# scychon/openmm_drudeNose

Hardware: AMD Instinct MI355X
Metric: integrator steps/sec at 1M Drude pairs (higher is better)
Workload: dtype f64; 1 GPU; SWM4-NDP water box, 1000000 molecules = 5000000 particle slots, 1000000 Drude pairs, 1 temperature group (+ molecular-COM and Drude thermostats), TGNH mode, mixed precision, numNHChains=1, hard wall 0.02 nm, harness force call-out inside the timed region (harness_force: lattice); harness_force=lattice, precision=mixed, variant=resident, hipgraph=False, parallelism=particle-sharded x1 (whole molecules), one KE all-reduce per step, slots_per_gpu=5000000

## Files before the change

### openmm_drudenose_amd/csrc/tgnh_context.h

```cpp
#ifndef TGNH_CONTEXT_H_
#define TGNH_CONTEXT_H_

#include <map>
#include <string>
#include <vector>

#include "tgnh_internal.h"
#include "tgnh_by_index.h"
#include "tgnh_minimize.h"

void tgnh_set_error(const std::string& msg);

namespace tgnh {
template <typename T> class DeviceBuf {
    T* p_ = nullptr;
    bool pinned_ = false;
public:
    DeviceBuf() = default;
    DeviceBuf(DeviceBuf&& o) noexcept : p_(o.p_), pinned_(o.pinned_) { o.p_ = nullptr; }
    DeviceBuf& operator=(DeviceBuf&& o) noexcept {
        if (this != &o) { reset(); p_ = o.p_; pinned_ = o.pinned_; o.p_ = nullptr; }
        return *this;
    }
    ~DeviceBuf() { reset(); }
// ... 24 lines not shown
    tgnh_status ensure(int grid, bool zero, const char* too_small);
};
}

struct tgnh_context {
    tgnh_desc d;
    int device = 0;
    bool host_only = false;
    struct Topology {
        std::vector<double> mass;
        std::vector<int> pair_drude, pair_parent, group, resid, normal;
        std::vector<int> res_count, res_first;
        std::vector<int> tile_start, tile_res;
        std::vector<int2> res_entries;
        std::vector<int> big_first, big_count;
        int num_big = 0, num_tiles = 0;
        std::vector<uint32_t> meta;
        std::vector<int2> wave_tile;
        std::vector<uint32_t> wmeta;
        std::vector<uint32_t> tile_pat, wtile_pat;
        std::vector<uint32_t> pattern, wpattern;
        std::vector<double> wpat_mass;
        bool wpat_all_uniform = false;
        int num_wtiles = 0;
        tgnh::DeviceBuf<uint32_t> d_meta, d_wmeta, d_tile_pat, d_pattern, d_wpattern;
        tgnh::DeviceBuf<int> d_tile_start, d_tile_res;
        tgnh::DeviceBuf<int2> d_res_table, d_wave_tile, d_big_table;
        tgnh::DeviceBytes d_big_com;
    } topo;
    struct Gather {
        bool generic = false;
        bool chain = false;
        std::string reason;
        std::vector<int2> res_table;
        std::vector<int> resid, partner;
        int com_lanes = 64;
        tgnh::DeviceBuf<int> d_group, d_resid, d_partner;
        tgnh::DeviceBuf<int2> d_res_table;
        tgnh::DeviceBytes d_com;
        tgnh::DeviceBuf<double> d_scratch;
    } gather;
    struct ByIndex {
        tgnh::DeviceBuf<int> d_partner;
    } by_index;
    tgnh::RowScratch<tgnh::DrudeStatsRow> dstats;
    struct CmMotion : tgnh::RowScratch<tgnh::CmRow> {
// ... 140 lines not shown
        tgnh::DeviceBuf<double> d_partials;
        tgnh::DeviceBuf<double> d_state;
        tgnh::DeviceBuf<double> d_stage;
        tgnh::DeviceBuf<double> d_scalar;
    } thermo;
    struct LaunchConfig {
        int grid = 0, gb = 1;
        int num_cus = 256, grid_override = 0;
        std::map<int, int> grid_cache;
        bool alternate_sweeps = true;
        int inline_sum_rows = tgnh::CHAIN_INLINE_SUM_ROWS;
        bool inline_sum_all = false;
        bool carry_ok = false;
        bool inline_chain = false;
        bool wave_ke = false;
        int resident_grid[5][2] = {{0, 0}, {0, 0}, {0, 0}, {0, 0}, {0, 0}};
        int resident_share = 1;
        int wresident_per_cu = 0, wresident_grid = 0;
        int resident_per_cu = 0;
    } cfg;
    struct VelPlanes {
        tgnh::DeviceBytes d_planes;
        tgnh::DeviceBytes d_invm;
        tgnh::DeviceBuf<uint32_t> d_mismatch;
        int verdict = 0;
        int streak = 0;
        bool pinned = false;
        hipStream_t stream = nullptr;
        bool usable() const { return d_planes.get() != nullptr && verdict >= 0 && !pinned; }
    } vp;
    struct Owed {
        bool end_pending = false;
        bool scale_pending = false;
        bool kick_pending = false;
        bool first_half_done = false;
        bool chain_pending = false;
        bool sum_pending = false;
        bool xwait_pending = false;
        bool stage_pending = false;
        bool ke_carry = false;
        bool planes_live = false;
        bool chain_pending_twice = false;
        bool carry_pending = false;
        bool tail_summed = false;
        bool end_folded = false;
        bool g_com_fresh = false;
// ... 80 lines not shown
```

### openmm_drudenose_amd/csrc/tgnh_internal.h

```cpp
#ifndef TGNH_INTERNAL_H_
#define TGNH_INTERNAL_H_

#include <hip/hip_runtime.h>
#include <stdint.h>
#include <type_traits>

#include "../../include/drude_tgnh.h"

namespace tgnh {

#ifndef TGNH_SPT
#define TGNH_SPT 2
#endif
#ifndef TGNH_TBLOCK
#define TGNH_TBLOCK 256
#endif
constexpr int BLOCK = 256;
constexpr int TBLOCK = TGNH_TBLOCK;
constexpr int SPT = TGNH_SPT;
constexpr int TILE_SLOTS = TBLOCK * SPT;
constexpr int TILE_RES = TILE_SLOTS / 2;
constexpr int GRID_CAP = 2048;
constexpr int MAX_GROUPS = 32;

// ... 116 lines not shown
    int num_wtiles;
    int tail_sum;
    double* ke_red;
    int num_tiles;
    int reverse;
    int padded;
    int num_groups;
    int use_com;
    int hardwall;
    double dt;
    double max_dist;
    double hw_scale;
    int chain_on;
    int sum_rows;
    int commit_len, commit_skip, commit_skip_n;
    const double* commit_src;
    double* commit_dst;
    int x_wait;
    const double* st_in;
    double* st_out;
    ChainArgs chain;
    void* vplanes;
    const void* wpat_invm;
};

struct BigComArgs {
    const int2* table;
    int n;
    const void* velm;
    const long long* force;
    int padded;
    int kick;
    double dt;
    void* big_com;
    double* partials;
    int NT, G;
};

struct ForceArgs {
    const void* posq;
    const void* posq_corr;
    const void* x0;
    const uint32_t* meta;
    long long* force;
    int n, padded;
    int reverse;
// ... 78 lines not shown
```

### openmm_drudenose_amd/csrc/tgnh_lifecycle.cpp

```cpp
#include <memory>

#include "tgnh_host.h"
#ifndef TGNH_MEETING_MEM
#define TGNH_MEETING_MEM hipDeviceMallocFinegrained
#endif

static thread_local std::string g_err;
extern "C" const char* tgnh_last_error(void) { return g_err.c_str(); }
extern "C" int tgnh_abi_version(void) { return TGNH_ABI_VERSION; }

void tgnh_set_error(const std::string& msg) { g_err = msg; }

static tgnh_status validate_desc(const tgnh_desc* d, bool* long_chain) {
    if (d->struct_size != sizeof(tgnh_desc)) return fail(TGNH_ERR_ARG, "tgnh_desc size mismatch (ABI)");
    if (d->mode != TGNH_MODE_DUALNH && d->mode != TGNH_MODE_TGNH) return fail(TGNH_ERR_ARG, "bad mode");
    if (d->precision < TGNH_PREC_SINGLE || d->precision > TGNH_PREC_DOUBLE) return fail(TGNH_ERR_ARG, "bad precision");
    if (d->num_particles < 1 || d->num_pairs < 0 || !d->mass || (d->num_pairs && (!d->pair_drude || !d->pair_parent)))
        return fail(TGNH_ERR_ARG, "bad particle / pair arrays");
    if (d->padded_num_particles < d->num_particles) return fail(TGNH_ERR_ARG, "padded_num_particles < num_particles");
    if (d->num_constraints < 0) return fail(TGNH_ERR_ARG, "negative num_constraints");
    if (3LL * d->padded_num_particles > 2147483647LL)
        return fail(TGNH_ERR_UNSUPPORTED, "more than 715 827 882 padded particle slots: the index into the third force plane leaves 32 bits");
    if (d->num_nh_chains < 1 || d->drude_steps_per_real_step < 1) return fail(TGNH_ERR_ARG, "numNHChains and drudeStepsPerRealStep must be >= 1");
    if (d->mode == TGNH_MODE_TGNH && (d->num_groups < 1 || d->num_residues < 1 || !d->group || !d->resid))
// ... 107 lines not shown
}

static tgnh_status resident_census(tgnh_context* c) {
    if (!(c->d.flags & TGNH_FLAG_RESIDENT_STEP) || c->cfg.gb == 0 || !c->cfg.inline_chain || c->thermo.L.NT > CHAIN_INLINE_SUM_NT) return TGNH_OK;
    const int kind = pass_kind(c->d);
    const size_t lds = tile_lds_bytes(c->d.precision, step_kind_ops2(kind), true, true);
    tgnh_status rc = census(c, c->thermo.L.C == 1 ? step_blocks_per_cu(c->d.precision, c->cfg.gb, kind, lds) : 0,
                            [&](const TileArgs& a, int grid) { return launch_step(c->d.precision, c->cfg.gb, kind, a, grid, lds, (hipStream_t)0); },
                            &c->cfg.resident_per_cu);
    if (rc) return rc;
    const bool multi = c->thermo.L.C > 1;
    bool want_w = c->cfg.wave_ke && (c->d.flags & TGNH_FLAG_DEFER_SCALE) && (c->cfg.resident_per_cu > 0 || multi);
    if (c->d.mode == TGNH_MODE_DUALNH && !c->thermo.L.use_drude_chains && multi) want_w = false;
#ifdef TGNH_TUNING
    if (const char* e = getenv("TGNH_WSTEP")) want_w = want_w && e[0] != '0';
#endif
    return census(c, want_w ? wstep_blocks_per_cu(c->d.precision, c->cfg.gb, multi) : 0,
                  [&](const TileArgs& a, int grid) { return launch_wstep(c->d.precision, c->cfg.gb, multi, a, grid, (hipStream_t)0); },
                  &c->cfg.wresident_per_cu);
}

static tgnh_status allocate_velocity_planes(tgnh_context* c) {
    if (const char* e = getenv("TGNH_VELOCITY_PLANES")) if (e[0] == '0') return TGNH_OK;
    if (!(c->d.flags & TGNH_FLAG_DEFER_SCALE) || c->cfg.wresident_per_cu <= 0 || !c->topo.wpat_all_uniform) return TGNH_OK;
    if (c->d.precision == TGNH_PREC_SINGLE) return TGNH_OK;
    if (wstep_blocks_per_cu(c->d.precision, c->cfg.gb, c->thermo.L.C > 1, true) < c->cfg.wresident_per_cu) return TGNH_OK;
    const bool single = c->d.precision == TGNH_PREC_SINGLE;
    const size_t word = single ? sizeof(float) : sizeof(double), n = c->topo.wpat_mass.size();
    std::vector<double> inv(n);
    for (size_t k = 0; k < n; k++) inv[k] = c->topo.wpat_mass[k] == 0.0 ? 0.0 : 1.0 / c->topo.wpat_mass[k];
    std::vector<float> inv_f(inv.begin(), inv.end());
    HIP_OK(c->vp.d_invm.upload(reinterpret_cast<const unsigned char*>(single ? (const void*)inv_f.data() : (const void*)inv.data()), n * word));
    HIP_OK(c->vp.d_mismatch.alloc(1, true));
    HIP_OK(c->vp.d_planes.alloc(3 * (size_t)c->d.padded_num_particles * word, true));
    return TGNH_OK;
}

extern "C" tgnh_status tgnh_create(const tgnh_desc* d, tgnh_handle* out) {
    if (!d || !out) return fail(TGNH_ERR_ARG, "null argument");
    bool long_chain = false;
    tgnh_status rc = validate_desc(d, &long_chain); if (rc) return rc;
    const bool host_only = d->device == -1;
    if (!host_only) {
        int ndev = 0;
        HIP_OK(hipGetDeviceCount(&ndev));
        if (d->device < 0 || d->device >= ndev) return fail(TGNH_ERR_HIP, "no such HIP device (the HIP path needs an MI355X; there is no CPU fallback)");
        HIP_OK(hipSetDevice(d->device));
    }

    std::unique_ptr<tgnh_context> owner(new tgnh_context());
    tgnh_context* c = owner.get();
    c->host_only = host_only;
    c->d = *d;
    c->device = d->device;
    set_bath_temperatures(c, d->temperature, d->drude_temperature);
    make_layout(c);
    c->cfg.gb = c->thermo.L.G <= 1 ? 1 : (c->thermo.L.G <= 4 ? 4 : (c->thermo.L.G <= 8 ? 8 : 0));
// ... 132 lines not shown
```

### openmm_drudenose_amd/csrc/tgnh_queries.cpp

```cpp
#include "tgnh_host.h"

static tgnh_status read_state(tgnh_handle h, int off, int n, hipStream_t s, double* out) {
    if (!out) return fail(TGNH_ERR_ARG, "null out");
    if (h->host_only) { std::copy(h->thermo.h_state.begin() + off, h->thermo.h_state.begin() + off + n, out); return TGNH_OK; }
    { tgnh_status rc = entry(h, false); if (rc) return rc; }
    { tgnh_status rc = materialize_chain(h, s); if (rc) return rc; }
    HIP_OK(hipMemcpyAsync(out, h->thermo.d_state + off, sizeof(double) * n, hipMemcpyDeviceToHost, s));
    return finish_query(h, s);
}

extern "C" tgnh_status tgnh_get_kinetic_energy(tgnh_handle h, int ke_sum_valid, void* stream, double* out) {
    CHECK_H(h);
    if (!out) return fail(TGNH_ERR_ARG, "null out");
    hipStream_t s = (hipStream_t)stream;
    if (h->d.mode == TGNH_MODE_TGNH && ke_sum_valid)
        return read_state(h, h->thermo.L.off_kesum, 1, s, out);
    tgnh_status rc = entry(h, true); if (rc) return rc;
    rc = flush_impl(h, s); if (rc) return rc;
    const double ts = h->d.mode == TGNH_MODE_DUALNH ? 0.5 * h->d.step_size : 0.0;
    HIP_OK(launch_plain_ke(h->d.precision, h->bound.velm, reinterpret_cast<const long long*>(h->bound.force), h->d.num_particles,
                           h->d.padded_num_particles, ts, h->thermo.d_scalar, s));
    HIP_OK(hipMemcpyAsync(out, h->thermo.d_scalar, sizeof(double), hipMemcpyDeviceToHost, s));
    HIP_OK(hipStreamSynchronize(s));
    return TGNH_OK;
// ... 77 lines not shown
        case 0: return &h->topo.normal;
        case 1: return &h->topo.pair_drude;
        case 2: return &h->topo.pair_parent;
        case 3: return &h->topo.group;
        case 4: return &h->topo.resid;
        case 5: return &h->topo.res_count;
        case 6: return &h->topo.res_first;
        case 7: return &h->topo.tile_start;
        default: return nullptr;
    }
}
extern "C" tgnh_status tgnh_get_topology_len(tgnh_handle h, int which, int* len) {
    CHECK_H(h);
    if (!len) return fail(TGNH_ERR_ARG, "null out");
    if (which == 8) { *len = (int)h->topo.meta.size(); return TGNH_OK; }
    if (which == 9) { *len = 2 * (int)h->topo.wave_tile.size(); return TGNH_OK; }
    if (which == 10) { *len = (int)h->topo.wmeta.size(); return TGNH_OK; }
    if (which == 11) { *len = (int)h->topo.tile_pat.size(); return TGNH_OK; }
    if (which == 12) { *len = (int)h->topo.wtile_pat.size(); return TGNH_OK; }
    if (which == 13) { *len = (int)h->topo.pattern.size(); return TGNH_OK; }
    if (which == 14) { *len = (int)h->topo.wpattern.size(); return TGNH_OK; }
    if (which == 15) { *len = 2 * (int)h->topo.wpat_mass.size(); return TGNH_OK; }
    if (which == 16) { *len = 1; return TGNH_OK; }
    const std::vector<int>* v = topo_vec(h, which);
    if (!v) return fail(TGNH_ERR_ARG, "bad topology array id");
    *len = (int)v->size();
    return TGNH_OK;
}
extern "C" tgnh_status tgnh_get_topology(tgnh_handle h, int which, int32_t* out) {
    CHECK_H(h);
    if (!out) return fail(TGNH_ERR_ARG, "null out");
    auto put = [&](const void* src, size_t bytes) { if (bytes) std::memcpy(out, src, bytes); return TGNH_OK; };
    if (which == 8) return put(h->topo.meta.data(), sizeof(uint32_t) * h->topo.meta.size());
    if (which == 9) return put(h->topo.wave_tile.data(), sizeof(int2) * h->topo.wave_tile.size());
    if (which == 10) return put(h->topo.wmeta.data(), sizeof(uint32_t) * h->topo.wmeta.size());
    if (which == 11) return put(h->topo.tile_pat.data(), sizeof(uint32_t) * h->topo.tile_pat.size());
    if (which == 12) return put(h->topo.wtile_pat.data(), sizeof(uint32_t) * h->topo.wtile_pat.size());
    if (which == 13) return put(h->topo.pattern.data(), sizeof(uint32_t) * h->topo.pattern.size());
    if (which == 14) return put(h->topo.wpattern.data(), sizeof(uint32_t) * h->topo.wpattern.size());
    if (which == 15) return put(h->topo.wpat_mass.data(), sizeof(double) * h->topo.wpat_mass.size());
    if (which == 16) { *out = h->topo.wpat_all_uniform ? 1 : 0; return TGNH_OK; }
    const std::vector<int>* v = topo_vec(h, which);
    if (!v) return fail(TGNH_ERR_ARG, "bad topology array id");
    std::copy(v->begin(), v->end(), out);
    return TGNH_OK;
}

extern "C" tgnh_status tgnh_compute_kinetic_energies(tgnh_handle h, void* stream) {
    tgnh_status rc = entry(h, true); if (rc) return rc;
    return ke_query_launches(h, (hipStream_t)stream);
}

tgnh_status ke_query_launches(tgnh_handle h, hipStream_t s) {
    tgnh_status rc = settle_kick(h, s); if (rc) return rc;
    rc = materialize_chain(h, s); if (rc) return rc;
    const int dir = h->run.sweep_reverse;
    rc = run_tile(h, OP_KE, KID_KE, s);
    h->run.sweep_reverse = dir;
    if (rc) return rc;
    if (h->gather.chain) {
        rc = run_chain_gather(h, s, true); if (rc) return rc;
    } else {
        ChainArgs a = chain_args(h);
        a.do_sum = 1; a.do_chain = 0;
// ... 104 lines not shown
```

### openmm_drudenose_amd/csrc/tgnh_step.cpp

```cpp
#include "tgnh_host.h"

constexpr int64_t STATUS_POLL_EVERY = 64;

void note_status(tgnh_handle h, uint32_t flags) {
    if (h->status.failed_code) return;
    if (flags & 8u) {
        h->status.failed_code = TGNH_ERR_STATE;
        h->status.failed = "resident step (noticed at step " + std::to_string((long long)h->run.step_count) + "): the launch's work-groups did "
                    "not all become resident within the time limit (TGNH_FLAG_RESIDENT_STEP needs the device to itself)";
        if (flags & 4u) h->status.failed += "; the waiting work-groups timed out in turn (status bits 2 and 3)";
    } else if (flags & 16u) {
        h->status.failed_code = TGNH_ERR_STATE;
        h->status.failed = "kinetic-energy pass (noticed at step " + std::to_string((long long)h->run.step_count) + "): work-group 0 did not "
                    "receive every work-group's row of sums within the time limit (the sums were left as NaN: nothing integrated "
                    "on with a partial sum); the device is shared with something that keeps this launch's work-groups from running "
                    "-- or a chain was handed a NaN kinetic energy: with an all-reduce attached, the rank on which that happened";
    } else if (flags & 4u) {
        h->status.failed_code = TGNH_ERR_STATE;
        h->status.failed = "mailbox exchange timed out (noticed at step " + std::to_string((long long)h->run.step_count) +
                    "): a peer did not send its kinetic-energy sums; the run cannot continue";
    } else if ((flags & 1u) && h->d.mode == TGNH_MODE_DUALNH) {
        h->status.failed_code = TGNH_ERR_HARDWALL;
        h->status.failed = "Drude particle moved too far beyond hard wall constraint";
    }
// ... 299 lines not shown
    if (kind == 0 && h->cfg.wresident_per_cu > 0) return 2;
    return h->cfg.resident_per_cu > 0 && h->thermo.L.C == 1 ? 1 : 0;
}
bool resident_now(tgnh_handle h) { return resident_kernel(h, pass_kind(h->d)) != 0; }

extern "C" tgnh_status tgnh_get_step_path(tgnh_handle h, int* gather, const char** reason) {
    CHECK_H(h);
    if (gather) *gather = h->gather.generic ? (h->gather.chain ? 2 : 1) : 0;
    if (reason) *reason = h->gather.reason.c_str();
    return TGNH_OK;
}

extern "C" tgnh_status tgnh_get_resident_kernel(tgnh_handle h, int* which) {
    CHECK_H(h);
    if (!which) return fail(TGNH_ERR_ARG, "null out");
    *which = resident_kernel(h, pass_kind(h->d));
    return TGNH_OK;
}

constexpr int PLANES_AFTER_STEPS = 8;

static tgnh_status leave_planes(tgnh_handle h, hipStream_t s) {
    if (!h->owed.planes_live) return TGNH_OK;
    HIP_OK(launch_planes_to_velm(h->d.precision, h->vp.d_planes, h->bound.velm, h->d.num_particles, h->d.padded_num_particles, s));
    h->owed.planes_live = false;
    return TGNH_OK;
}

static tgnh_status enter_planes(tgnh_handle h, hipStream_t s) {
    tgnh_context::VelPlanes& vp = h->vp;
    if (h->owed.planes_live || !vp.usable()) return TGNH_OK;
    if (stream_capturing(s)) { vp.pinned = true; return TGNH_OK; }
    if (vp.streak < PLANES_AFTER_STEPS) return TGNH_OK;
    const bool check = vp.verdict == 0;
    if (check) HIP_OK(hipMemsetAsync(vp.d_mismatch, 0, sizeof(uint32_t), s));
    HIP_OK(launch_velm_to_planes(h->d.precision, h->bound.velm, vp.d_planes, h->topo.d_wave_tile, h->topo.num_wtiles, vp.d_invm,
                                 h->d.padded_num_particles, check ? vp.d_mismatch.get() : nullptr, s));
    if (check) {
        uint32_t differs = 1;
        HIP_OK(hipMemcpyAsync(&differs, vp.d_mismatch, sizeof(uint32_t), hipMemcpyDeviceToHost, s));
        HIP_OK(hipStreamSynchronize(s));
        vp.verdict = differs ? -1 : 1;
        if (differs) return TGNH_OK;
    }
    h->owed.planes_live = true;
    return TGNH_OK;
}

tgnh_status velm_current(tgnh_handle h, hipStream_t s) {
    return h->owed.planes_live && !h->owed.end_pending ? settle_end(h, s) : TGNH_OK;
}

extern "C" tgnh_status tgnh_get_velocity_planes(tgnh_handle h, int32_t out[4]) {
    CHECK_H(h);
    if (!out) return fail(TGNH_ERR_ARG, "null out");
    out[0] = h->owed.planes_live ? 1 : 0; out[1] = h->vp.usable() ? 1 : 0; out[2] = h->vp.streak; out[3] = PLANES_AFTER_STEPS;
    return TGNH_OK;
}

static tgnh_status run_resident(tgnh_handle h, hipStream_t s, int kind) {
    if (h->owed.stage_pending) { tgnh_status rc = commit_stage(h, s); if (rc) return rc; }
    const bool wstep = resident_kernel(h, kind) == 2;
    if (wstep && kind == 0) { tgnh_status rc = enter_planes(h, s); if (rc) return rc; }
    else if (h->owed.planes_live) return fail(TGNH_ERR_STATE, "internal: a launch that reads velm while the velocities live in the planes");
    TileArgs a = tile_args(h, nullptr);
    if (h->owed.planes_live) { a.vplanes = h->vp.d_planes; a.wpat_invm = h->vp.d_invm; h->vp.stream = s; }
    const int ops2 = step_kind_ops2(kind);
    if ((ops2 & OP_POSDELTA) && !h->bound.pos_delta) return fail(TGNH_ERR_STATE, "posDelta buffer not bound");
    const bool hw = a.hardwall != 0 && (ops2 & (OP_DRIFT | OP_MOVE));
    const size_t lds = tile_lds_bytes(h->d.precision, ops2, hw, a.use_com != 0);
    int& grid = h->cfg.resident_grid[kind][hw ? 1 : 0];
    if (grid == 0 && !wstep) {
        int per_cu = std::min(h->cfg.resident_per_cu, step_blocks_per_cu(h->d.precision, h->cfg.gb, kind, lds));
        if (per_cu < 1) return fail(TGNH_ERR_HIP, "step_kernel: occupancy query failed");
        grid = std::max(1, std::min(std::min(h->topo.num_tiles, per_cu * h->cfg.num_cus / h->cfg.resident_share), GRID_CAP));
    }
    a.chain_on = 1;
    a.chain = chain_args(h);
    a.chain.chain_twice = kind == 0 ? 1 : 0;
    a.x_wait = 1;
    if (!h->xchg.on) a.chain.x = h->meet.self_x;
    a.st_in = h->thermo.d_state; a.st_out = h->thermo.d_state;
    a.sync = h->meet.d_sync; a.rows = h->meet.d_rows;
    if (big_com_on(h)) { tgnh_status rc = run_big_com(h, kind == 0 || kind == 2, s); if (rc) return rc; }
    if (wstep && h->cfg.wresident_grid == 0) {
        const int need = (h->topo.num_wtiles + WBLOCK / 64 - 1) / (WBLOCK / 64);
        h->cfg.wresident_grid = std::max(1, std::min(std::min(need, h->cfg.wresident_per_cu * h->cfg.num_cus / h->cfg.resident_share), GRID_CAP));
    }
    const int g = wstep ? h->cfg.wresident_grid : grid;
// ... 207 lines not shown
```

### openmm_drudenose_amd/csrc/tgnh_topology.cpp

```cpp
#include <map>

#include "tgnh_host.h"

std::vector<int> partner_table(const tgnh_context* c) {
    std::vector<int> t(c->d.num_particles, -1);
    for (size_t k = 0; k < c->topo.pair_drude.size(); k++) {
        const int p = c->topo.pair_drude[k], p1 = c->topo.pair_parent[k];
        t[p] = (int)((unsigned)p1 | 0x80000000u); t[p1] = p;
    }
    return t;
}
tgnh_status device_partner_table(tgnh_context* c, const int** out) {
    if (!c->gather.d_partner && !c->by_index.d_partner) HIP_OK(c->by_index.d_partner.upload(partner_table(c)));
    *out = c->gather.d_partner ? c->gather.d_partner : c->by_index.d_partner;
    return TGNH_OK;
}

static tgnh_status build_gather_topology(tgnh_context* c, const std::vector<int>& res_order) {
    const tgnh_desc& d = c->d;
    const int N = d.num_particles;
    const bool com = com_thermostat_on(d);
    c->topo.tile_start.assign(1, N); c->topo.tile_res.assign(1, 0); c->topo.num_tiles = 0;
    c->topo.res_entries.assign(1, make_int2(0, 0));
    c->topo.meta.clear(); c->topo.wave_tile.clear(); c->topo.wmeta.clear(); c->topo.num_wtiles = 0;
// ... 263 lines not shown
                if (intern(ids, c->topo.pattern, c->topo.meta.data() + ts, P, 1u << 16, &id))
                    c->topo.tile_pat[t] = (uint32_t)P | (mols << 8) | (id << 16);
                break;
            }
        }
        c->topo.wtile_pat.assign(std::max(c->topo.num_wtiles, 1), 0u); c->topo.wpattern.clear(); c->topo.wpat_mass.clear();
        c->topo.wpat_all_uniform = c->topo.num_wtiles > 0;
        for (int t = 0; t < c->topo.num_wtiles; t++) {
            const int ws = c->topo.wave_tile[t].x, n = c->topo.wave_tile[t + 1].x - ws;
            for (int P = 1; P <= PATTERN_WORDS && P <= n; P++) {
                bool same = true;
                for (int k = 0; k < n && same; k++) same = c->topo.wmeta[ws + k] == c->topo.wmeta[ws + k % P];
                if (!same) continue;
                uint32_t id;
                if (intern(wids, c->topo.wpattern, c->topo.wmeta.data() + ws, P, 1u << 16, &id, c->topo.mass.data() + ws, P == n)) {
                    c->topo.wtile_pat[t] = (uint32_t)P | (id << 8);
                    for (int k = 0; k < n; k++)
                        if (std::memcmp(&c->topo.mass[ws + k], &c->topo.wpat_mass[(size_t)id * PATTERN_WORDS + k % P], sizeof(double))) c->topo.wpat_all_uniform = false;
                }
                break;
            }
            if (!c->topo.wtile_pat[t]) c->topo.wpat_all_uniform = false;
        }
        if (c->topo.pattern.empty()) c->topo.pattern.assign(PATTERN_WORDS, 0u);
        if (c->topo.wpattern.empty()) c->topo.wpattern.assign(PATTERN_WORDS, 0u);
    }
    if (c->host_only) return TGNH_OK;
    HIP_OK(c->topo.d_tile_pat.upload(c->topo.tile_pat));
    HIP_OK(c->topo.d_pattern.upload(c->topo.pattern));
    HIP_OK(c->topo.d_wpattern.upload(c->topo.wpattern));
    HIP_OK(c->topo.d_meta.upload(c->topo.meta));
    HIP_OK(c->topo.d_tile_start.upload(c->topo.tile_start));
    HIP_OK(c->topo.d_tile_res.upload(c->topo.tile_res));
    HIP_OK(c->topo.d_res_table.upload(c->topo.res_entries));
    if (!c->topo.wave_tile.empty()) {
        std::vector<int2> packed = c->topo.wave_tile;
        for (int t = 0; t < c->topo.num_wtiles; t++) packed[t].y |= (int)(c->topo.wtile_pat[t] << 8);
        HIP_OK(c->topo.d_wave_tile.upload(packed));
        HIP_OK(c->topo.d_wmeta.upload(c->topo.wmeta));
    }
    if (c->topo.num_big) {
        std::vector<int2> bt(c->topo.num_big);
        for (int k = 0; k < c->topo.num_big; k++) bt[k] = make_int2(c->topo.big_count[k], c->topo.big_first[k]);
        HIP_OK(c->topo.d_big_table.upload(bt));
        HIP_OK(c->topo.d_big_com.alloc(32 * (size_t)c->topo.num_big, true));
    }
// ... 174 lines not shown
```

### openmm_drudenose_amd/csrc/tgnh_vplanes.h

```cpp
#ifndef TGNH_VPLANES_H_
#define TGNH_VPLANES_H_

#include "tgnh_internal.h"

namespace tgnh {

hipError_t launch_velm_to_planes(int precision, const void* velm, void* planes, const int2* wave_tile, int num_wtiles,
                                 const void* wpat_invm, int padded, uint32_t* mismatch, hipStream_t s);
hipError_t launch_planes_to_velm(int precision, const void* planes, void* velm, int n, int padded, hipStream_t s);

}

#endif
```

### openmm_drudenose_amd/csrc/tgnh_vplanes.hip

```cpp
#include "tgnh_vplanes.h"
#include "tgnh_device_math.h"

namespace tgnh {

__device__ __forceinline__ bool same_bits(const float a, const float b) { return __float_as_uint(a) == __float_as_uint(b); }
__device__ __forceinline__ bool same_bits(const double a, const double b) { return __double_as_longlong(a) == __double_as_longlong(b); }

template <int PREC>
__global__ __launch_bounds__(BLOCK) void velm_to_planes_kernel(const void* __restrict__ velm_, void* __restrict__ planes_, const int2* __restrict__ wave_tile,
                                                               const int num_wtiles, const void* __restrict__ invm_, const int padded,
                                                               uint32_t* __restrict__ mismatch) {
    typedef typename Prec<PREC>::mixed mixed;
    typedef typename Prec<PREC>::mixed4 mixed4;
    const int lane = (int)threadIdx.x & 63;
    const int t = (int)blockIdx.x * (BLOCK / 64) + ((int)threadIdx.x >> 6);
    if (t >= num_wtiles) return;
    const int ws = wave_tile[t].x, n = wave_tile[t + 1].x - ws;
    if (lane >= n) return;
    const int idx = ws + lane;
    const mixed4 v = reinterpret_cast<const mixed4*>(velm_)[idx];
    mixed* __restrict__ planes = reinterpret_cast<mixed*>(planes_);
    planes[idx] = v.x; planes[idx + padded] = v.y; planes[idx + 2 * padded] = v.z;
    if (mismatch) {
        const uint32_t p = (uint32_t)wave_tile[t].y >> 8;
        const int period = (int)(p & 255u);
        bool same = false;
        if (period) same = same_bits(reinterpret_cast<const mixed*>(invm_)[(p >> 8) * PATTERN_WORDS + (uint32_t)(lane % period)], v.w);
        if (!same) atomicOr(mismatch, 1u);
    }
}

template <int PREC>
__global__ __launch_bounds__(BLOCK) void planes_to_velm_kernel(const void* __restrict__ planes_, void* __restrict__ velm_, const int n, const int padded) {
    typedef typename Prec<PREC>::mixed mixed;
    typedef typename Prec<PREC>::mixed4 mixed4;
    const mixed* __restrict__ planes = reinterpret_cast<const mixed*>(planes_);
    mixed4* __restrict__ velm = reinterpret_cast<mixed4*>(velm_);
    const long long i = (long long)blockIdx.x * BLOCK + threadIdx.x;
    if (i >= n) return;
    mixed4 v = velm[i];
    v.x = planes[i]; v.y = planes[i + padded]; v.z = planes[i + 2ll * padded];
    velm[i] = v;
}

hipError_t launch_velm_to_planes(int precision, const void* velm, void* planes, const int2* wave_tile, int num_wtiles,
                                 const void* wpat_invm, int padded, uint32_t* mismatch, hipStream_t s) {
    if (!velm || !planes || !wave_tile || !wpat_invm || num_wtiles < 1 || padded < 1) return hipErrorInvalidValue;
    const int grid = (num_wtiles + BLOCK / 64 - 1) / (BLOCK / 64);
    TGNH_LAUNCH_PREC(velm_to_planes_kernel, precision, dim3(grid), dim3(BLOCK), 0, s, velm, planes, wave_tile, num_wtiles, wpat_invm, padded, mismatch);
    return hipGetLastError();
}

hipError_t launch_planes_to_velm(int precision, const void* planes, void* velm, int n, int padded, hipStream_t s) {
    if (!velm || !planes || n < 1 || padded < n) return hipErrorInvalidValue;
    const int grid = (n + BLOCK - 1) / BLOCK;
    TGNH_LAUNCH_PREC(planes_to_velm_kernel, precision, dim3(grid), dim3(BLOCK), 0, s, planes, velm, n, padded);
    return hipGetLastError();
}

}
```

### openmm_drudenose_amd/csrc/tgnh_wave_device.h

```cpp
#ifndef TGNH_WAVE_DEVICE_H_
#define TGNH_WAVE_DEVICE_H_
#include "tgnh_tile_device.h"

namespace tgnh {

struct PatternWord {
    uint32_t pat = 0u, word = 0u;
    template <typename Also>
    __device__ __forceinline__ bool of(const TileArgs& a, const uint32_t p, const int lane, Also&& also) {
        if ((p & 255u) == 0u) return false;
        if (p != pat) {
            const int period = (int)(p & 255u);
            const int q = (int)(((float)lane + 0.5f) * __builtin_amdgcn_rcpf((float)period));
            const uint32_t at = (p >> 8) * PATTERN_WORDS + (uint32_t)(lane - q * period);
            word = a.wpattern[at];
            also(at);
            pat = p;
        }
        return true;
    }
    __device__ __forceinline__ bool of(const TileArgs& a, const uint32_t p, const int lane) { return of(a, p, lane, [](uint32_t) {}); }
};

template <int PREC> struct WaveIn {
// ... 13 lines not shown
    long long fx = 0, fy = 0, fz = 0;
    if (lane < n) {
        v = velm[idx];
        if (!patterned) meta = a.wmeta[idx];
        if (OPS & OP_KICK) {
            fx = a.force[idx];
            fy = a.force[idx + a.padded];
            fz = a.force[idx + 2 * a.padded];
        }
    }
    if (patterned && lane < n) meta = pword;
    in.v = v; in.meta = meta; in.fx = fx; in.fy = fy; in.fz = fz;
}

template <int PREC> struct WStepIn {
    typename Prec<PREC>::mixed4 v;
    uint32_t meta;
    long long fx, fy, fz;
    typename Prec<PREC>::real4 p;
    float4 c;
    typename Prec<PREC>::mixed mass, cx, cy, cz;
};

struct WaveBounds { int ws, y, n; };

template <int PREC, int GB, bool PLANES = false> struct WaveStep {
    typedef typename Prec<PREC>::real real;
    typedef typename Prec<PREC>::mixed mixed;
    typedef typename Prec<PREC>::real4 real4;
    typedef typename Prec<PREC>::mixed4 mixed4;
    const TileArgs& a;
    TileEnv<PREC, GB>* e;
    const double* s_scale;
    mixed *ix, *iy, *iz, *im, *jx, *jy, *jz;
    mixed4* __restrict__ velm; real4* __restrict__ posq; float4* __restrict__ pcorr;
    mixed* __restrict__ vpl;
    mixed pinvm;
    int lane, G, nw;
    bool use_com, hardwall;
    mixed dt, fscale;
    PatternWord pw;
    __device__ __forceinline__ WaveStep(const TileArgs& a_, TileEnv<PREC, GB>* e_, const double* s_scale_, mixed* img, const int lane_)
        : a(a_), e(e_), s_scale(s_scale_), ix(img), iy(img + WAVE_SLOTS), iz(img + 2 * WAVE_SLOTS), im(img + 3 * WAVE_SLOTS),
          jx(img + 4 * WAVE_SLOTS), jy(img + 5 * WAVE_SLOTS), jz(img + 6 * WAVE_SLOTS),
          velm(reinterpret_cast<mixed4*>(a_.velm)), posq(reinterpret_cast<real4*>(a_.posq)), pcorr(reinterpret_cast<float4*>(a_.posq_corr)),
          vpl(reinterpret_cast<mixed*>(a_.vplanes)), pinvm((mixed)0), lane(lane_), G(a_.num_groups), nw(a_.num_wtiles), use_com(a_.use_com != 0), hardwall(a_.hardwall != 0),
          dt((mixed)a_.dt), fscale((mixed)(0.5 * a_.dt / 4294967296.0)) {}
    __device__ __forceinline__ static void wfence() {
        __builtin_amdgcn_fence(__ATOMIC_RELEASE, "wavefront");
        __builtin_amdgcn_wave_barrier();
        __builtin_amdgcn_fence(__ATOMIC_ACQUIRE, "wavefront");
    }
    __device__ __forceinline__ void bounds(const int ww, WaveBounds& b) const {
        const int2* t = a.wave_tile + (a.reverse ? nw - 1 - ww : ww);
        b.ws = t[0].x; b.y = t[0].y; b.n = t[1].x - b.ws;
    }
    __device__ __forceinline__ void load_vf(const WaveBounds& b, WStepIn<PREC>& in) {
        const int idx = b.ws + lane;
        const bool patterned = pw.of(a, (uint32_t)b.y >> 8, lane, [&](const uint32_t at) {
            if (PLANES) pinvm = reinterpret_cast<const mixed*>(a.wpat_invm)[at];
        });
        mixed4 v = mk4((mixed)0, (mixed)0, (mixed)0, (mixed)0);
        uint32_t meta = 64u << 10;
        long long fx = 0, fy = 0, fz = 0;
        if (lane < b.n) {
            if (PLANES) v = mk4(vpl[idx], vpl[idx + a.padded], vpl[idx + 2 * a.padded], pinvm);
            else v = reinterpret_cast<const mixed4*>(a.velm)[idx];
            if (!patterned) meta = a.wmeta[idx];
            fx = a.force[idx]; fy = a.force[idx + a.padded]; fz = a.force[idx + 2 * a.padded];
        }
        if (patterned && lane < b.n) meta = pw.word;
        in.v = v; in.meta = meta; in.fx = fx; in.fy = fy; in.fz = fz;
    }
    __device__ __forceinline__ void load_x(const WaveBounds& b, WStepIn<PREC>& in) const {
        const int idx = b.ws + lane;
        if (lane < b.n) {
            in.p = reinterpret_cast<const real4*>(a.posq)[idx];
            if (PREC == TGNH_PREC_MIXED) in.c = reinterpret_cast<const float4*>(a.posq_corr)[idx];
        }
    }
    template <bool KICK = true>
    __device__ __forceinline__ void prepare(WStepIn<PREC>& t, const WaveBounds& bd, const bool ke) {
        mixed4& v = t.v;
        const uint32_t m = t.meta;
        t.mass = v.w != 0 ? rcp_(v.w) : (mixed)0;
        if (KICK) {
            const mixed c = fscale * v.w;
            v.x += c * force_as(t.fx, (mixed)0);
            v.y += c * force_as(t.fy, (mixed)0);
            v.z += c * force_as(t.fz, (mixed)0);
// ... 100 lines not shown
                    dotvr2 -= vbCMass;
                    if (dotvr1 != dotvr2) deltaT = deltaR / abs_(dotvr1 - dotvr2);
                    if (deltaT > dt) deltaT = dt;
                    const mixed vBond = hws / sqrt_(mass1);
                    dotvr1 = -dotvr1 * vBond * mass2 * invTot / abs_(dotvr1);
                    dotvr2 = -dotvr2 * vBond * mass1 * invTot / abs_(dotvr2);
                    const mixed dr1 = -deltaR * mass2 * invTot + deltaT * dotvr1;
                    const mixed dr2 = deltaR * mass1 * invTot + deltaT * dotvr2;
                    dotvr1 += vbCMass;
                    dotvr2 += vbCMass;
                    if (is_d) {
                        px += bx * dr1; py += by * dr1; pz += bz * dr1;
                        v.x = vp1x + bx * dotvr1; v.y = vp1y + by * dotvr1; v.z = vp1z + bz * dotvr1;
                    } else {
                        px += bx * dr2; py += by * dr2; pz += bz * dr2;
                        v.x = vp2x + bx * dotvr2; v.y = vp2y + by * dotvr2; v.z = vp2z + bz * dotvr2;
                    }
                }
            }
        }
        wfence();
        if (lane < bd.n) {
            const int idx = bd.ws + lane;
            if (PLANES) { vpl[idx] = v.x; vpl[idx + a.padded] = v.y; vpl[idx + 2 * a.padded] = v.z; }
            else velm[idx] = v;
            store_position<PREC>(posq, pcorr, idx, px, py, pz, pq);
        }
    }
};

}
#endif
```

Measured before the change: 4474 steps/s.

## Compact velocity planes to store only massive particles per wave tile

Velocity planes now hold only particles with nonzero mass (skipping SWM4 virtual sites), packed per wave tile with 16-aligned bases and per-pattern lane offsets. This cuts the plane footprint and the traffic of the velocity reads and writes in the wave step and in the conversion kernels. In exchange, each lane does extra index lookups (tile base, pattern offset) and the scatter is somewhat less contiguous. The verdict check now also requires massless slots to hold finite velocities.

```diff
diff --git a/openmm_drudenose_amd/csrc/tgnh_context.h b/openmm_drudenose_amd/csrc/tgnh_context.h
--- a/openmm_drudenose_amd/csrc/tgnh_context.h
+++ b/openmm_drudenose_amd/csrc/tgnh_context.h
@@ -70,6 +70,7 @@
         std::vector<uint32_t> pattern, wpattern;
         std::vector<double> wpat_mass;
         bool wpat_all_uniform = false;
+        std::vector<uint32_t> wtile_base, wpat_off;
         int num_wtiles = 0;
         tgnh::DeviceBuf<uint32_t> d_meta, d_wmeta, d_tile_pat, d_pattern, d_wpattern;
         tgnh::DeviceBuf<int> d_tile_start, d_tile_res;
@@ -256,6 +257,8 @@
     struct VelPlanes {
         tgnh::DeviceBytes d_planes;
         tgnh::DeviceBytes d_invm;
+        tgnh::DeviceBuf<uint32_t> d_base, d_off;
+        int stride = 0;
         tgnh::DeviceBuf<uint32_t> d_mismatch;
         int verdict = 0;
         int streak = 0;
diff --git a/openmm_drudenose_amd/csrc/tgnh_internal.h b/openmm_drudenose_amd/csrc/tgnh_internal.h
--- a/openmm_drudenose_amd/csrc/tgnh_internal.h
+++ b/openmm_drudenose_amd/csrc/tgnh_internal.h
@@ -162,6 +162,9 @@
     ChainArgs chain;
     void* vplanes;
     const void* wpat_invm;
+    const uint32_t* wtile_base;
+    const uint32_t* wpat_off;
+    int vstride;
 };
 
 struct BigComArgs {
diff --git a/openmm_drudenose_amd/csrc/tgnh_lifecycle.cpp b/openmm_drudenose_amd/csrc/tgnh_lifecycle.cpp
--- a/openmm_drudenose_amd/csrc/tgnh_lifecycle.cpp
+++ b/openmm_drudenose_amd/csrc/tgnh_lifecycle.cpp
@@ -153,7 +153,7 @@
 
 static tgnh_status allocate_velocity_planes(tgnh_context* c) {
     if (const char* e = getenv("TGNH_VELOCITY_PLANES")) if (e[0] == '0') return TGNH_OK;
-    if (!(c->d.flags & TGNH_FLAG_DEFER_SCALE) || c->cfg.wresident_per_cu <= 0 || !c->topo.wpat_all_uniform) return TGNH_OK;
+    if (!(c->d.flags & TGNH_FLAG_DEFER_SCALE) || c->cfg.wresident_per_cu <= 0 || !c->topo.wpat_all_uniform || c->topo.wtile_base.empty()) return TGNH_OK;
     if (c->d.precision == TGNH_PREC_SINGLE) return TGNH_OK;
     if (wstep_blocks_per_cu(c->d.precision, c->cfg.gb, c->thermo.L.C > 1, true) < c->cfg.wresident_per_cu) return TGNH_OK;
     const bool single = c->d.precision == TGNH_PREC_SINGLE;
@@ -163,7 +163,10 @@
     std::vector<float> inv_f(inv.begin(), inv.end());
     HIP_OK(c->vp.d_invm.upload(reinterpret_cast<const unsigned char*>(single ? (const void*)inv_f.data() : (const void*)inv.data()), n * word));
     HIP_OK(c->vp.d_mismatch.alloc(1, true));
-    HIP_OK(c->vp.d_planes.alloc(3 * (size_t)c->d.padded_num_particles * word, true));
+    c->vp.stride = (int)c->topo.wtile_base.back();
+    HIP_OK(c->vp.d_base.upload(c->topo.wtile_base));
+    HIP_OK(c->vp.d_off.upload(c->topo.wpat_off));
+    HIP_OK(c->vp.d_planes.alloc(3 * (size_t)std::max(c->vp.stride, 1) * word, true));
     return TGNH_OK;
 }
 
diff --git a/openmm_drudenose_amd/csrc/tgnh_queries.cpp b/openmm_drudenose_amd/csrc/tgnh_queries.cpp
--- a/openmm_drudenose_amd/csrc/tgnh_queries.cpp
+++ b/openmm_drudenose_amd/csrc/tgnh_queries.cpp
@@ -123,6 +123,7 @@
     if (which == 14) { *len = (int)h->topo.wpattern.size(); return TGNH_OK; }
     if (which == 15) { *len = 2 * (int)h->topo.wpat_mass.size(); return TGNH_OK; }
     if (which == 16) { *len = 1; return TGNH_OK; }
+    if (which == 17) { *len = 2 + (int)h->topo.wtile_base.size() + (int)h->topo.wpat_off.size(); return TGNH_OK; }
     const std::vector<int>* v = topo_vec(h, which);
     if (!v) return fail(TGNH_ERR_ARG, "bad topology array id");
     *len = (int)v->size();
@@ -141,6 +142,13 @@
     if (which == 14) return put(h->topo.wpattern.data(), sizeof(uint32_t) * h->topo.wpattern.size());
     if (which == 15) return put(h->topo.wpat_mass.data(), sizeof(double) * h->topo.wpat_mass.size());
     if (which == 16) { *out = h->topo.wpat_all_uniform ? 1 : 0; return TGNH_OK; }
+    if (which == 17) {
+        const std::vector<uint32_t>&base = h->topo.wtile_base, &off = h->topo.wpat_off;
+        out[0] = base.empty() ? 0 : (int32_t)base.back(); out[1] = (int32_t)base.size();
+        if (!base.empty()) std::memcpy(out + 2, base.data(), sizeof(uint32_t) * base.size());
+        if (!off.empty()) std::memcpy(out + 2 + base.size(), off.data(), sizeof(uint32_t) * off.size());
+        return TGNH_OK;
+    }
     const std::vector<int>* v = topo_vec(h, which);
     if (!v) return fail(TGNH_ERR_ARG, "bad topology array id");
     std::copy(v->begin(), v->end(), out);
diff --git a/openmm_drudenose_amd/csrc/tgnh_step.cpp b/openmm_drudenose_amd/csrc/tgnh_step.cpp
--- a/openmm_drudenose_amd/csrc/tgnh_step.cpp
+++ b/openmm_drudenose_amd/csrc/tgnh_step.cpp
@@ -345,7 +345,8 @@
 
 static tgnh_status leave_planes(tgnh_handle h, hipStream_t s) {
     if (!h->owed.planes_live) return TGNH_OK;
-    HIP_OK(launch_planes_to_velm(h->d.precision, h->vp.d_planes, h->bound.velm, h->d.num_particles, h->d.padded_num_particles, s));
+    HIP_OK(launch_planes_to_velm(h->d.precision, h->vp.d_planes, h->bound.velm, h->topo.d_wave_tile, h->topo.num_wtiles, h->vp.d_invm,
+                                 h->vp.d_base, h->vp.d_off, h->vp.stride, s));
     h->owed.planes_live = false;
     return TGNH_OK;
 }
@@ -358,7 +359,7 @@
     const bool check = vp.verdict == 0;
     if (check) HIP_OK(hipMemsetAsync(vp.d_mismatch, 0, sizeof(uint32_t), s));
     HIP_OK(launch_velm_to_planes(h->d.precision, h->bound.velm, vp.d_planes, h->topo.d_wave_tile, h->topo.num_wtiles, vp.d_invm,
-                                 h->d.padded_num_particles, check ? vp.d_mismatch.get() : nullptr, s));
+                                 vp.d_base, vp.d_off, vp.stride, check ? vp.d_mismatch.get() : nullptr, s));
     if (check) {
         uint32_t differs = 1;
         HIP_OK(hipMemcpyAsync(&differs, vp.d_mismatch, sizeof(uint32_t), hipMemcpyDeviceToHost, s));
@@ -387,7 +388,10 @@
     if (wstep && kind == 0) { tgnh_status rc = enter_planes(h, s); if (rc) return rc; }
     else if (h->owed.planes_live) return fail(TGNH_ERR_STATE, "internal: a launch that reads velm while the velocities live in the planes");
     TileArgs a = tile_args(h, nullptr);
-    if (h->owed.planes_live) { a.vplanes = h->vp.d_planes; a.wpat_invm = h->vp.d_invm; h->vp.stream = s; }
+    if (h->owed.planes_live) {
+        a.vplanes = h->vp.d_planes; a.wpat_invm = h->vp.d_invm; a.wtile_base = h->vp.d_base; a.wpat_off = h->vp.d_off; a.vstride = h->vp.stride;
+        h->vp.stream = s;
+    }
     const int ops2 = step_kind_ops2(kind);
     if ((ops2 & OP_POSDELTA) && !h->bound.pos_delta) return fail(TGNH_ERR_STATE, "posDelta buffer not bound");
     const bool hw = a.hardwall != 0 && (ops2 & (OP_DRIFT | OP_MOVE));
diff --git a/openmm_drudenose_amd/csrc/tgnh_topology.cpp b/openmm_drudenose_amd/csrc/tgnh_topology.cpp
--- a/openmm_drudenose_amd/csrc/tgnh_topology.cpp
+++ b/openmm_drudenose_amd/csrc/tgnh_topology.cpp
@@ -309,6 +309,32 @@
             }
             if (!c->topo.wtile_pat[t]) c->topo.wpat_all_uniform = false;
         }
+        c->topo.wtile_base.clear(); c->topo.wpat_off.clear();
+        if (c->topo.wpat_all_uniform) {
+            const size_t patterns = c->topo.wpattern.size() / PATTERN_WORDS;
+            std::vector<char> made(patterns, 0);
+            c->topo.wpat_off.assign(patterns * PATTERN_WORDS, 0u);
+            c->topo.wtile_base.assign((size_t)c->topo.num_wtiles + 1, 0u);
+            uint64_t base = 0;
+            for (int t = 0; t < c->topo.num_wtiles; t++) {
+                const int ws = c->topo.wave_tile[t].x, n = c->topo.wave_tile[t + 1].x - ws;
+                const uint32_t P = c->topo.wtile_pat[t] & 255u, id = c->topo.wtile_pat[t] >> 8;
+                if (!made[id]) {
+                    uint32_t before = 0;
+                    for (uint32_t lane = 0; lane < (uint32_t)PATTERN_WORDS; lane++) {
+                        c->topo.wpat_off[(size_t)id * PATTERN_WORDS + lane] = before;
+                        before += c->topo.wpat_mass[(size_t)id * PATTERN_WORDS + lane % P] != 0.0;
+                    }
+                    made[id] = 1;
+                }
+                uint32_t massive = 0;
+                for (int k = 0; k < n; k++) massive += c->topo.mass[ws + k] != 0.0;
+                c->topo.wtile_base[t] = (uint32_t)base;
+                base = (base + massive + 15u) & ~(uint64_t)15u;
+            }
+            c->topo.wtile_base[c->topo.num_wtiles] = (uint32_t)base;
+            if (3 * base > (uint64_t)INT32_MAX) { c->topo.wtile_base.clear(); c->topo.wpat_off.clear(); }
+        }
         if (c->topo.pattern.empty()) c->topo.pattern.assign(PATTERN_WORDS, 0u);
         if (c->topo.wpattern.empty()) c->topo.wpattern.assign(PATTERN_WORDS, 0u);
     }
diff --git a/openmm_drudenose_amd/csrc/tgnh_vplanes.h b/openmm_drudenose_amd/csrc/tgnh_vplanes.h
--- a/openmm_drudenose_amd/csrc/tgnh_vplanes.h
+++ b/openmm_drudenose_amd/csrc/tgnh_vplanes.h
@@ -6,8 +6,10 @@
 namespace tgnh {
 
 hipError_t launch_velm_to_planes(int precision, const void* velm, void* planes, const int2* wave_tile, int num_wtiles,
-                                 const void* wpat_invm, int padded, uint32_t* mismatch, hipStream_t s);
-hipError_t launch_planes_to_velm(int precision, const void* planes, void* velm, int n, int padded, hipStream_t s);
+                                 const void* wpat_invm, const uint32_t* wtile_base, const uint32_t* wpat_off, int stride,
+                                 uint32_t* mismatch, hipStream_t s);
+hipError_t launch_planes_to_velm(int precision, const void* planes, void* velm, const int2* wave_tile, int num_wtiles,
+                                 const void* wpat_invm, const uint32_t* wtile_base, const uint32_t* wpat_off, int stride, hipStream_t s);
 
 }
 
diff --git a/openmm_drudenose_amd/csrc/tgnh_vplanes.hip b/openmm_drudenose_amd/csrc/tgnh_vplanes.hip
--- a/openmm_drudenose_amd/csrc/tgnh_vplanes.hip
+++ b/openmm_drudenose_amd/csrc/tgnh_vplanes.hip
@@ -5,56 +5,83 @@
 
 __device__ __forceinline__ bool same_bits(const float a, const float b) { return __float_as_uint(a) == __float_as_uint(b); }
 __device__ __forceinline__ bool same_bits(const double a, const double b) { return __double_as_longlong(a) == __double_as_longlong(b); }
+template <typename T> __device__ __forceinline__ bool finite3(const T x, const T y, const T z) { return x - x == (T)0 && y - y == (T)0 && z - z == (T)0; }
+
+template <typename mixed> struct PlaneSlot {
+    int idx, word;
+    mixed invm;
+    bool inside, patterned;
+    __device__ __forceinline__ PlaneSlot(const int2* __restrict__ wave_tile, const int num_wtiles, const void* __restrict__ invm_,
+                                         const uint32_t* __restrict__ base, const uint32_t* __restrict__ off) {
+        const int lane = (int)threadIdx.x & 63;
+        const int t = (int)blockIdx.x * (BLOCK / 64) + ((int)threadIdx.x >> 6);
+        inside = false; patterned = false; idx = 0; word = 0; invm = (mixed)0;
+        if (t >= num_wtiles) return;
+        const int ws = wave_tile[t].x, n = wave_tile[t + 1].x - ws;
+        if (lane >= n) return;
+        inside = true;
+        idx = ws + lane;
+        const uint32_t p = (uint32_t)wave_tile[t].y >> 8;
+        const int period = (int)(p & 255u);
+        if (!period) return;
+        patterned = true;
+        invm = reinterpret_cast<const mixed*>(invm_)[(p >> 8) * PATTERN_WORDS + (uint32_t)(lane % period)];
+        word = (int)(base[t] + off[(p >> 8) * PATTERN_WORDS + (uint32_t)lane]);
+    }
+};
 
 template <int PREC>
 __global__ __launch_bounds__(BLOCK) void velm_to_planes_kernel(const void* __restrict__ velm_, void* __restrict__ planes_, const int2* __restrict__ wave_tile,
-                                                               const int num_wtiles, const void* __restrict__ invm_, const int padded,
-                                                               uint32_t* __restrict__ mismatch) {
+                                                               const int num_wtiles, const void* __restrict__ invm_, const uint32_t* __restrict__ base,
+                                                               const uint32_t* __restrict__ off, const int stride, uint32_t* __restrict__ mismatch) {
     typedef typename Prec<PREC>::mixed mixed;
     typedef typename Prec<PREC>::mixed4 mixed4;
-    const int lane = (int)threadIdx.x & 63;
-    const int t = (int)blockIdx.x * (BLOCK / 64) + ((int)threadIdx.x >> 6);
-    if (t >= num_wtiles) return;
-    const int ws = wave_tile[t].x, n = wave_tile[t + 1].x - ws;
-    if (lane >= n) return;
-    const int idx = ws + lane;
-    const mixed4 v = reinterpret_cast<const mixed4*>(velm_)[idx];
+    const PlaneSlot<mixed> s(wave_tile, num_wtiles, invm_, base, off);
+    if (!s.inside) return;
+    const mixed4 v = reinterpret_cast<const mixed4*>(velm_)[s.idx];
     mixed* __restrict__ planes = reinterpret_cast<mixed*>(planes_);
-    planes[idx] = v.x; planes[idx + padded] = v.y; planes[idx + 2 * padded] = v.z;
+    if (s.patterned && s.invm != (mixed)0) { planes[s.word] = v.x; planes[s.word + stride] = v.y; planes[s.word + 2 * stride] = v.z; }
     if (mismatch) {
-        const uint32_t p = (uint32_t)wave_tile[t].y >> 8;
-        const int period = (int)(p & 255u);
-        bool same = false;
-        if (period) same = same_bits(reinterpret_cast<const mixed*>(invm_)[(p >> 8) * PATTERN_WORDS + (uint32_t)(lane % period)], v.w);
+        bool same = s.patterned && same_bits(s.invm, v.w);
+        if (same && s.invm == (mixed)0) same = finite3(v.x, v.y, v.z);
         if (!same) atomicOr(mismatch, 1u);
     }
 }
 
 template <int PREC>
-__global__ __launch_bounds__(BLOCK) void planes_to_velm_kernel(const void* __restrict__ planes_, void* __restrict__ velm_, const int n, const int padded) {
+__global__ __launch_bounds__(BLOCK) void planes_to_velm_kernel(const void* __restrict__ planes_, void* __restrict__ velm_, const int2* __restrict__ wave_tile,
+                                                               const int num_wtiles, const void* __restrict__ invm_, const uint32_t* __restrict__ base,
+                                                               const uint32_t* __restrict__ off, const int stride) {
     typedef typename Prec<PREC>::mixed mixed;
     typedef typename Prec<PREC>::mixed4 mixed4;
+    const PlaneSlot<mixed> s(wave_tile, num_wtiles, invm_, base, off);
+    if (!s.inside || !s.patterned || s.invm == (mixed)0) return;
     const mixed* __restrict__ planes = reinterpret_cast<const mixed*>(planes_);
     mixed4* __restrict__ velm = reinterpret_cast<mixed4*>(velm_);
-    const long long i = (long long)blockIdx.x * BLOCK + threadIdx.x;
-    if (i >= n) return;
-    mixed4 v = velm[i];
-    v.x = planes[i]; v.y = planes[i + padded]; v.z = planes[i + 2ll * padded];
-    velm[i] = v;
+    mixed4 v = velm[s.idx];
+    v.x = planes[s.word]; v.y = planes[s.word + stride]; v.z = planes[s.word + 2 * stride];
+    velm[s.idx] = v;
+}
+
+static bool planes_args_ok(const void* velm, const void* planes, const int2* wave_tile, int num_wtiles, const void* wpat_invm,
+                           const uint32_t* wtile_base, const uint32_t* wpat_off, int stride) {
+    return velm && planes && wave_tile && wpat_invm && wtile_base && wpat_off && num_wtiles >= 1 && stride >= 1;
 }
 
 hipError_t launch_velm_to_planes(int precision, const void* velm, void* planes, const int2* wave_tile, int num_wtiles,
-                                 const void* wpat_invm, int padded, uint32_t* mismatch, hipStream_t s) {
-    if (!velm || !planes || !wave_tile || !wpat_invm || num_wtiles < 1 || padded < 1) return hipErrorInvalidValue;
+                                 const void* wpat_invm, const uint32_t* wtile_base, const uint32_t* wpat_off, int stride,
+                                 uint32_t* mismatch, hipStream_t s) {
+    if (!planes_args_ok(velm, planes, wave_tile, num_wtiles, wpat_invm, wtile_base, wpat_off, stride)) return hipErrorInvalidValue;
     const int grid = (num_wtiles + BLOCK / 64 - 1) / (BLOCK / 64);
-    TGNH_LAUNCH_PREC(velm_to_planes_kernel, precision, dim3(grid), dim3(BLOCK), 0, s, velm, planes, wave_tile, num_wtiles, wpat_invm, padded, mismatch);
+    TGNH_LAUNCH_PREC(velm_to_planes_kernel, precision, dim3(grid), dim3(BLOCK), 0, s, velm, planes, wave_tile, num_wtiles, wpat_invm, wtile_base, wpat_off, stride, mismatch);
     return hipGetLastError();
 }
 
-hipError_t launch_planes_to_velm(int precision, const void* planes, void* velm, int n, int padded, hipStream_t s) {
-    if (!velm || !planes || n < 1 || padded < n) return hipErrorInvalidValue;
-    const int grid = (n + BLOCK - 1) / BLOCK;
-    TGNH_LAUNCH_PREC(planes_to_velm_kernel, precision, dim3(grid), dim3(BLOCK), 0, s, planes, velm, n, padded);
+hipError_t launch_planes_to_velm(int precision, const void* planes, void* velm, const int2* wave_tile, int num_wtiles,
+                                 const void* wpat_invm, const uint32_t* wtile_base, const uint32_t* wpat_off, int stride, hipStream_t s) {
+    if (!planes_args_ok(velm, planes, wave_tile, num_wtiles, wpat_invm, wtile_base, wpat_off, stride)) return hipErrorInvalidValue;
+    const int grid = (num_wtiles + BLOCK / 64 - 1) / (BLOCK / 64);
+    TGNH_LAUNCH_PREC(planes_to_velm_kernel, precision, dim3(grid), dim3(BLOCK), 0, s, planes, velm, wave_tile, num_wtiles, wpat_invm, wtile_base, wpat_off, stride);
     return hipGetLastError();
 }
 
diff --git a/openmm_drudenose_amd/csrc/tgnh_wave_device.h b/openmm_drudenose_amd/csrc/tgnh_wave_device.h
--- a/openmm_drudenose_amd/csrc/tgnh_wave_device.h
+++ b/openmm_drudenose_amd/csrc/tgnh_wave_device.h
@@ -59,7 +59,7 @@
     typename Prec<PREC>::mixed mass, cx, cy, cz;
 };
 
-struct WaveBounds { int ws, y, n; };
+struct WaveBounds { int ws, y, n, base; };
 
 template <int PREC, int GB, bool PLANES = false> struct WaveStep {
     typedef typename Prec<PREC>::real real;
@@ -73,6 +73,7 @@
     mixed4* __restrict__ velm; real4* __restrict__ posq; float4* __restrict__ pcorr;
     mixed* __restrict__ vpl;
     mixed pinvm;
+    int poff;
     int lane, G, nw;
     bool use_com, hardwall;
     mixed dt, fscale;
@@ -81,7 +82,7 @@
         : a(a_), e(e_), s_scale(s_scale_), ix(img), iy(img + WAVE_SLOTS), iz(img + 2 * WAVE_SLOTS), im(img + 3 * WAVE_SLOTS),
           jx(img + 4 * WAVE_SLOTS), jy(img + 5 * WAVE_SLOTS), jz(img + 6 * WAVE_SLOTS),
           velm(reinterpret_cast<mixed4*>(a_.velm)), posq(reinterpret_cast<real4*>(a_.posq)), pcorr(reinterpret_cast<float4*>(a_.posq_corr)),
-          vpl(reinterpret_cast<mixed*>(a_.vplanes)), pinvm((mixed)0), lane(lane_), G(a_.num_groups), nw(a_.num_wtiles), use_com(a_.use_com != 0), hardwall(a_.hardwall != 0),
+          vpl(reinterpret_cast<mixed*>(a_.vplanes)), pinvm((mixed)0), poff(0), lane(lane_), G(a_.num_groups), nw(a_.num_wtiles), use_com(a_.use_com != 0), hardwall(a_.hardwall != 0),
           dt((mixed)a_.dt), fscale((mixed)(0.5 * a_.dt / 4294967296.0)) {}
     __device__ __forceinline__ static void wfence() {
         __builtin_amdgcn_fence(__ATOMIC_RELEASE, "wavefront");
@@ -89,20 +90,29 @@
         __builtin_amdgcn_fence(__ATOMIC_ACQUIRE, "wavefront");
     }
     __device__ __forceinline__ void bounds(const int ww, WaveBounds& b) const {
-        const int2* t = a.wave_tile + (a.reverse ? nw - 1 - ww : ww);
+        const int at = a.reverse ? nw - 1 - ww : ww;
+        const int2* t = a.wave_tile + at;
         b.ws = t[0].x; b.y = t[0].y; b.n = t[1].x - b.ws;
+        if (PLANES) b.base = (int)a.wtile_base[at];
     }
     __device__ __forceinline__ void load_vf(const WaveBounds& b, WStepIn<PREC>& in) {
         const int idx = b.ws + lane;
         const bool patterned = pw.of(a, (uint32_t)b.y >> 8, lane, [&](const uint32_t at) {
-            if (PLANES) pinvm = reinterpret_cast<const mixed*>(a.wpat_invm)[at];
+            if (PLANES) {
+                pinvm = reinterpret_cast<const mixed*>(a.wpat_invm)[at];
+                poff = (int)a.wpat_off[((uint32_t)b.y >> 16) * PATTERN_WORDS + (uint32_t)lane];
+            }
         });
         mixed4 v = mk4((mixed)0, (mixed)0, (mixed)0, (mixed)0);
         uint32_t meta = 64u << 10;
         long long fx = 0, fy = 0, fz = 0;
         if (lane < b.n) {
-            if (PLANES) v = mk4(vpl[idx], vpl[idx + a.padded], vpl[idx + 2 * a.padded], pinvm);
-            else v = reinterpret_cast<const mixed4*>(a.velm)[idx];
+            if (PLANES) {
+                if (pinvm != (mixed)0) {
+                    const int vi = b.base + poff;
+                    v = mk4(vpl[vi], vpl[vi + a.vstride], vpl[vi + 2 * a.vstride], pinvm);
+                }
+            } else v = reinterpret_cast<const mixed4*>(a.velm)[idx];
             if (!patterned) meta = a.wmeta[idx];
             fx = a.force[idx]; fy = a.force[idx + a.padded]; fz = a.force[idx + 2 * a.padded];
         }
@@ -249,8 +259,12 @@
         wfence();
         if (lane < bd.n) {
             const int idx = bd.ws + lane;
-            if (PLANES) { vpl[idx] = v.x; vpl[idx + a.padded] = v.y; vpl[idx + 2 * a.padded] = v.z; }
-            else velm[idx] = v;
+            if (PLANES) {
+                if (pinvm != (mixed)0) {
+                    const int vi = bd.base + poff;
+                    vpl[vi] = v.x; vpl[vi + a.vstride] = v.y; vpl[vi + 2 * a.vstride] = v.z;
+                }
+            } else velm[idx] = v;
             store_position<PREC>(posq, pcorr, idx, px, py, pz, pq);
         }
     }
```

Result: faster. 4783 steps/s (median of 6 runs) (+6.9%).
